# MIT-SPARK/Khronos

Hardware: AMD Instinct MI355X
Metric: active-window frames/sec (+ Mvoxel-updates/sec) at 1280x720 RGB-D+labels, 2 cm voxels (higher is better)
Workload: dtype f32

## Files before the change

### khronos_amd/csrc/khr_kernels_objects.h

```cpp
#pragma once
#include "khr_device.h"

namespace khr {

constexpr int kGvWindow = 32766;
constexpr uint32_t kGvMaxGroup = 32766;
constexpr uint32_t kNodeNone = 0xffffffffu, kNodeOwner = 0x80000000u;

__host__ __device__ inline uint64_t gvKey(uint32_t group, int rx, int ry, int rz) {
  return (static_cast<uint64_t>(group) << 48) | (static_cast<uint64_t>(static_cast<uint32_t>(rx + 32768) & 0xffffu) << 32) |
         (static_cast<uint64_t>(static_cast<uint32_t>(ry + 32768) & 0xffffu) << 16) |
         static_cast<uint64_t>(static_cast<uint32_t>(rz + 32768) & 0xffffu);
}
__host__ __device__ inline uint64_t gvOriginKey(uint32_t group) { return static_cast<uint64_t>(group) << 48; }
__host__ __device__ inline bool gvIsOrigin(uint64_t k) { return (k & 0xffffffffffffull) == 0ull; }
__host__ __device__ inline void gvUnpack(uint64_t k, uint32_t* group, int* rx, int* ry, int* rz) {
  *group = static_cast<uint32_t>(k >> 48);
  *rx = static_cast<int>((k >> 32) & 0xffffu) - 32768;
  *ry = static_cast<int>((k >> 16) & 0xffffu) - 32768;
  *rz = static_cast<int>(k & 0xffffu) - 32768;
}

struct GvTable {
  uint64_t* keys;
// ... 9 lines not shown
    h = (h + 1) & t.mask;
  }
  return -1;
}
__device__ inline uint32_t gvInsert(const GvTable& t, uint64_t key, bool* claimed) {
  uint32_t h = hashKey(key) & t.mask;
  while (true) {
    const unsigned long long prev = atomicCAS(reinterpret_cast<unsigned long long*>(&t.keys[h]),
                                              static_cast<unsigned long long>(kEmptyKey), static_cast<unsigned long long>(key));
    if (prev == kEmptyKey) { *claimed = true; return h; }
    if (prev == key) { *claimed = false; return h; }
    h = (h + 1) & t.mask;
  }
}

__device__ inline uint32_t gvInsertWave(const GvTable& t, bool has, uint64_t key, bool* claimed) {
  const uint32_t lane = laneId();
  const uint32_t klo = static_cast<uint32_t>(key), khi = static_cast<uint32_t>(key >> 32);
  const uint32_t plo = __shfl_up(klo, 1), phi = __shfl_up(khi, 1);
  const unsigned long long hm = __ballot(has);
  const bool prev_has = lane > 0u && ((hm >> (lane - 1u)) & 1ull);
  const bool start = has && !(prev_has && plo == klo && phi == khi);
  const unsigned long long sm = __ballot(start);
  uint32_t h = 0;
  bool cl = false;
  if (start) h = gvInsert(t, key, &cl);
  *claimed = cl;
  const unsigned long long below = sm & (lane == 63u ? ~0ull : ((2ull << lane) - 1ull));
  const int src = below ? 63 - __clzll(static_cast<long long>(below)) : 0;
  const uint32_t hs = __shfl(h, src);
  return has ? hs : 0u;
}

__global__ __launch_bounds__(256) void k_gv_clear(uint64_t* __restrict__ keys, uint32_t n, uint32_t* __restrict__ counters) {
  const uint32_t i = blockIdx.x * blockDim.x + threadIdx.x;
  if (2 * i + 1 < n) reinterpret_cast<ulonglong2*>(keys)[i] = make_ulonglong2(kEmptyKey, kEmptyKey);
  else if (2 * i < n) keys[2 * i] = kEmptyKey;
  if (i < 4) counters[i] = 0u;
}

__device__ inline void pixelVertex(const DevFrame& f, int i, float* pw) {
  pw[0] = pw[1] = pw[2] = 0.f;
  if (f.range[i] > 0.f) {
    const float d = f.depth[i];
    const int u = i % f.W, v = i / f.W;
    xform(f.Rw, f.tw, ((static_cast<float>(u) - f.cx) / f.fx) * d, ((static_cast<float>(v) - f.cy) / f.fy) * d, d, pw);
  }
}

__device__ inline bool gvVoxelKey(const float* pw, float inv, int3 o, uint32_t group, bool vertex_is_origin, uint64_t* key) {
  const int rx = static_cast<int>(floorf(pw[0] * inv)) - o.x, ry = static_cast<int>(floorf(pw[1] * inv)) - o.y,
            rz = static_cast<int>(floorf(pw[2] * inv)) - o.z;
// ... 21 lines not shown
  return -1;
}

struct ObjAcc {
  uint32_t n_pixels;
  uint32_t first_cm;
  int32_t bmin[3], bmax[3];
  float sum[3];
  uint32_t group;
};

__global__ __launch_bounds__(256) void k_obj_insert3d(DevFrame f, const int32_t* __restrict__ obj_labels, int n_labels,
                                                     float max_range, float inv, int3 origin, GvTable t,
                                                     uint32_t* __restrict__ parent, uint32_t* __restrict__ pix_node,
                                                     uint32_t* __restrict__ flags ,
                                                     uint32_t* __restrict__ owners, uint32_t* __restrict__ n_owners) {
  const int i = blockIdx.x * blockDim.x + threadIdx.x;
  const bool in = i < f.W * f.H;
  bool has = false;
  uint64_t key = 0;
  if (in) {
    const int g = labelRank(obj_labels, n_labels, f.label[i]);
    const float r = f.range[i];
    if (g >= 0 && !(max_range > 0.f && r > max_range)) {
      float pw[3];
      pixelVertex(f, i, pw);
      has = gvVoxelKey(pw, inv, origin, static_cast<uint32_t>(g), !(r > 0.f), &key);
      if (!has) atomicOr(&flags[0], 1u);
    }
  }
  bool claimed;
  const uint32_t h = gvInsertWave(t, has, key, &claimed);
  const uint32_t at = waveAggInc(n_owners, claimed);
  if (claimed) {
    parent[h] = h;
    owners[at] = h;
  }
  if (in) pix_node[i] = has ? (h | (claimed ? kNodeOwner : 0u)) : kNodeNone;
}

__constant__ int8_t c_obj_fwd13[13][3] = {{1, 0, 0},  {0, 1, 0},   {0, 0, 1},  {1, 1, 0},  {-1, 1, 0}, {1, 0, 1}, {-1, 0, 1},
                                          {0, 1, 1},  {0, -1, 1},  {1, 1, 1},  {-1, 1, 1}, {1, -1, 1}, {-1, -1, 1}};

__global__ __launch_bounds__(256) void k_obj_union3d(const uint32_t* __restrict__ owners, const uint32_t* __restrict__ n_owners, GvTable t,
                                                    uint32_t* __restrict__ parent, int n_dirs) {
  const uint32_t total = *n_owners * static_cast<uint32_t>(n_dirs);
  for (uint32_t i = blockIdx.x * blockDim.x + threadIdx.x; i < total; i += gridDim.x * blockDim.x) {
    const uint32_t h = owners[i / n_dirs];
    const int k = static_cast<int>(i % n_dirs);
    const uint64_t key = t.keys[h];
    if (gvIsOrigin(key)) continue;
    uint32_t g;
    int x, y, z;
    gvUnpack(key, &g, &x, &y, &z);
    const int nx = x + c_obj_fwd13[k][0], ny = y + c_obj_fwd13[k][1], nz = z + c_obj_fwd13[k][2];
    if (nx < -kGvWindow || nx > kGvWindow || ny < -kGvWindow || ny > kGvWindow || nz < -kGvWindow || nz > kGvWindow) continue;
    const int hn = gvFind(t, gvKey(g, nx, ny, nz));
    if (hn >= 0) ufUnion(parent, h, static_cast<uint32_t>(hn));
  }
}

__global__ __launch_bounds__(256) void k_obj_roots3d(const uint32_t* __restrict__ owners, const uint32_t* __restrict__ n_owners,
                                                    uint32_t* __restrict__ parent, uint32_t* __restrict__ root_idx,
                                                    uint32_t* __restrict__ n_roots, uint32_t cap, ObjAcc* __restrict__ acc,
                                                    const uint64_t* __restrict__ keys) {
  const uint32_t i = blockIdx.x * blockDim.x + threadIdx.x;
  const bool on = i < *n_owners;
  uint32_t h = 0;
  bool is_root = false;
  if (on) {
    h = owners[i];
    const uint32_t r = ufFind(parent, h);
    is_root = r == h;
    if (!is_root) __atomic_store_n(parent + h, r, __ATOMIC_RELAXED);
  }
  const uint32_t idx = waveAggInc(n_roots, is_root);
  if (is_root) {
    root_idx[h] = idx;
    if (idx < cap) {
      ObjAcc a;
      a.n_pixels = 0;
      a.first_cm = 0xffffffffu;
      for (int d = 0; d < 3; ++d) { a.bmin[d] = INT32_MAX; a.bmax[d] = INT32_MIN; a.sum[d] = 0.f; }
      a.group = static_cast<uint32_t>(keys[h] >> 48);
      acc[idx] = a;
    }
  }
}

__global__ __launch_bounds__(256) void k_gv_release(const uint32_t* __restrict__ slots, const uint32_t* __restrict__ n_slots,
                                                   uint64_t* __restrict__ keys) {
  const uint32_t n = *n_slots;
  for (uint32_t i = blockIdx.x * blockDim.x + threadIdx.x; i < n; i += gridDim.x * blockDim.x) keys[slots[i]] = kEmptyKey;
}

__global__ __launch_bounds__(256) void k_gv_release_publish(const uint32_t* __restrict__ slots, const uint32_t* __restrict__ n_slots,
                                                           uint64_t* __restrict__ keys, uint32_t* __restrict__ done_count,
                                                           const uint32_t* __restrict__ src, volatile uint32_t* __restrict__ dst_host,
                                                           uint32_t rec_words, uint32_t max_recs, volatile uint32_t* __restrict__ ticket_host,
                                                           uint32_t ticket, uint32_t* __restrict__ counters_to_zero) {
  __shared__ uint32_t s_last;
// ... 2 lines not shown
  __syncthreads();
  if (threadIdx.x == 0) {
    __threadfence();
    s_last = atomicAdd(done_count, 1u) == gridDim.x - 1u ? 1u : 0u;
  }
  __syncthreads();
  if (!s_last) return;
  const uint32_t n_words = 4u + min(src[0], max_recs) * rec_words;
  for (uint32_t i = threadIdx.x; i < n_words; i += blockDim.x) dst_host[i] = src[i];
  __threadfence_system();
  __syncthreads();
  if (threadIdx.x < 4) counters_to_zero[threadIdx.x] = 0u;
  if (threadIdx.x == 0) {
    *done_count = 0u;
    *ticket_host = ticket;
    __threadfence_system();
  }
}

__global__ __launch_bounds__(256) void k_obj_init2d(DevFrame f, const int32_t* __restrict__ obj_labels, int n_labels,
                                                   uint32_t* __restrict__ parent, uint32_t* __restrict__ pix_node) {
  const int i = blockIdx.x * blockDim.x + threadIdx.x;
  if (i >= f.W * f.H) return;
  const bool cand = labelRank(obj_labels, n_labels, f.label[i]) >= 0;
  parent[i] = static_cast<uint32_t>(i);
  pix_node[i] = cand ? (static_cast<uint32_t>(i) | kNodeOwner) : kNodeNone;
}

__global__ __launch_bounds__(256) void k_obj_union2d(DevFrame f, const uint32_t* __restrict__ pix_node,
                                                    uint32_t* __restrict__ parent, int full) {
// ... 35 lines not shown
  if (is_root) {
    root_idx[h] = idx;
    if (idx < cap) {
      ObjAcc a;
      a.n_pixels = 0;
      a.first_cm = 0xffffffffu;
      for (int d = 0; d < 3; ++d) { a.bmin[d] = INT32_MAX; a.bmax[d] = INT32_MIN; a.sum[d] = 0.f; }
      a.group = keys3d ? static_cast<uint32_t>(keys3d[h] >> 48)
                       : static_cast<uint32_t>(labelRank(obj_labels, n_labels, label2d[h]));
      acc[idx] = a;
    }
  }
}

constexpr int kObjTile = 32, kObjSlots = 16;
__global__ __launch_bounds__(1024) void k_obj_paint(DevFrame f, const uint32_t* __restrict__ pix_node,
                                                   const uint32_t* __restrict__ parent, const uint32_t* __restrict__ root_idx,
                                                   uint32_t cap, int32_t* __restrict__ obj, ObjAcc* __restrict__ acc) {
  __shared__ int s_id[kObjSlots];
  __shared__ ObjAcc s_acc[kObjSlots];
  if (threadIdx.x < kObjSlots) {
    s_id[threadIdx.x] = 0;
    ObjAcc a;
    a.n_pixels = 0;
    a.first_cm = 0xffffffffu;
    for (int d = 0; d < 3; ++d) { a.bmin[d] = INT32_MAX; a.bmax[d] = INT32_MIN; a.sum[d] = 0.f; }
    a.group = 0;
    s_acc[threadIdx.x] = a;
  }
  __syncthreads();
  const int tiles_x = (f.W + kObjTile - 1) / kObjTile;
  const int u = (blockIdx.x % tiles_x) * kObjTile + (threadIdx.x & 31), v = (blockIdx.x / tiles_x) * kObjTile + (threadIdx.x >> 5);
  int id = 0;
  float pw[3] = {0.f, 0.f, 0.f};
  uint32_t cm = 0xffffffffu;
  if (u < f.W && v < f.H) {
    const int i = v * f.W + u;
    const uint32_t node = pix_node[i];
    if (node != kNodeNone) {
      const uint32_t idx = root_idx[ufFind(parent, node & ~kNodeOwner)];
      if (idx < cap) {
        id = static_cast<int>(idx) + 1;
        pixelVertex(f, i, pw);
        cm = static_cast<uint32_t>(u) * static_cast<uint32_t>(f.H) + static_cast<uint32_t>(v);
      }
    }
    obj[i] = id;
  }
  unsigned long long todo = __ballot(id != 0);
  while (todo) {
    const int leader = __ffsll(static_cast<long long>(todo)) - 1;
    const int cid = __shfl(id, leader);
    const bool mine = id == cid;
    const unsigned long long grp = __ballot(mine);
    todo &= ~grp;
    float mn[3], mx[3], sm[3];
    uint32_t first = mine ? cm : 0xffffffffu;
#pragma unroll
    for (int c = 0; c < 3; ++c) {
      mn[c] = mine ? pw[c] : 3.0e38f;
      mx[c] = mine ? pw[c] : -3.0e38f;
      sm[c] = mine ? pw[c] : 0.f;
// ... 37 lines not shown
#pragma unroll
    for (int c = 0; c < 3; ++c) {
      atomicMin(&a->bmin[c], l.bmin[c]);
      atomicMax(&a->bmax[c], l.bmax[c]);
      atomicAdd(&a->sum[c], l.sum[c]);
    }
  }
}

__global__ __launch_bounds__(256) void k_obj_remap(int32_t* __restrict__ obj, int n, const int32_t* __restrict__ final_id) {
  const int i = blockIdx.x * blockDim.x + threadIdx.x;
  if (i >= n) return;
  const int32_t t = obj[i];
  if (t) obj[i] = final_id[t - 1];
}
constexpr int kRemapTab = 256;
struct RemapTab {
  int32_t v[kRemapTab];
};
__global__ __launch_bounds__(256) void k_obj_remap_tab(int32_t* __restrict__ obj, int n, RemapTab tab) {
  __shared__ int32_t s_tab[kRemapTab];
  s_tab[threadIdx.x] = tab.v[threadIdx.x];
  __syncthreads();
  const int i = blockIdx.x * blockDim.x + threadIdx.x;
  if (i >= n) return;
  const int32_t t = obj[i];
  if (t) obj[i] = s_tab[t - 1];
}

__global__ __launch_bounds__(256) void k_cluster_voxels(DevFrame f, const int32_t* __restrict__ id_image, float inv, int3 origin,
                                                       GvTable t, uint64_t* __restrict__ list, uint32_t* __restrict__ n_list,
// ... 46 lines not shown
          pixelVertex(f, i, pw);
          has = gvVoxelKey(pw, inv, origin, static_cast<uint32_t>(id), !(f.range[i] > 0.f), &key);
          if (!has) atomicOr(&flags[0], 1u);
        }
      }
    }
  }
  bool claimed;
  const uint32_t h = gvInsertWave(t, has, key, &claimed);
  const uint32_t at = waveAggInc(n_list, claimed);
  if (claimed && at < cap) {
    list[at] = key;
    slots[at] = h;
  }
}


constexpr int kPixRefs = 32;
struct PixRefs {
  int n;
  int32_t id[kPixRefs];
  int32_t bit[kPixRefs];
};
struct PixCamera {
  double T[12];
  float fx, fy, cx, cy;
  int W, H;
};
__global__ __launch_bounds__(256) void k_pix_reproject(DevFrame src, const int32_t* __restrict__ id_img, PixRefs refs, PixCamera cam,
                                                      uint32_t* __restrict__ mask, uint32_t* __restrict__ n_points) {
  const int i = blockIdx.x * blockDim.x + threadIdx.x;
// ... 169 lines not shown
```

### khronos_amd/csrc/khronos_amd.hip

```cpp
#include <hip/hip_runtime.h>
#include <hip/hip_ext.h>
#include <hipcub/hipcub.hpp>

#include <algorithm>
#include <array>
#include <atomic>
#include <chrono>
#include <memory>
#include <mutex>
#include <cmath>
#include <cstdarg>
#include <cstdio>
#include <climits>
#include <cstring>
#include <cstdlib>
#include <functional>
#include <map>
#include <string>
#include <thread>
#include <tuple>
#include <unordered_map>
#include <vector>

#include "../../include/khronos_amd.h"
// ... 69 lines not shown
  bool dyn_clean = false;
  bool dynw_valid = false;
  uint64_t aux_seq = 0;
  std::vector<khr_cluster> sem_clusters;
  std::vector<khr_cluster> clusters;
};

struct TimingRec {
  int which;
  Event a, b;
};

constexpr int kNumTimers = 13;
constexpr uint32_t kObjHead = 512;
constexpr uint32_t kCvHead = 8192;
constexpr int kGvReleaseGrid = 64;
constexpr uint32_t kCompCap = 1024, kCompHead = 64;

}

struct khr_ctx {
  khr_config cfg{};
  DevParams p{};
  DevMap m{};
  int device = 0;
  Stream stream;
  Stream aux_stream;
  Stream copy_stream;
  Stream snap_stream;
  Stream mc_stream;
// ... 172 lines not shown
  size_t cub_temp_bytes = 0;
  bool obj_configured = false;
  khr_object_detector_config obj_cfg{};
  std::vector<int32_t> obj_labels;
  DevBuf<int32_t> d_obj_labels;
  uint64_t* d_gv_keys = nullptr;
  uint32_t gv_mask = 0;
  uint32_t *d_gv_parent = nullptr, *d_gv_rootidx = nullptr, *d_gv_node = nullptr;
  uint32_t* d_gv_n = nullptr;
  ObjAcc* d_obj_acc = nullptr;
  int32_t* d_obj_final = nullptr;
  uint64_t* d_cv_list = nullptr;
  uint32_t obj_root_cap = 0;
  uint32_t* d_gv_owners = nullptr;
  uint32_t* d_gv_done = nullptr;
  bool gv_clean = false;
  bool gv_counters_clean[4] = {false, false, false, false};
  PinnedBuf<uint8_t> h_obj_head;
  Event ev_obj;
  int obj_pending_slot = -1;
  uint32_t* d_cv_n[3] = {nullptr, nullptr, nullptr};
  uint64_t* d_cv_keys[3] = {nullptr, nullptr, nullptr};
  PinnedBuf<uint8_t> h_cv[3];
  Event ev_cv[3];
  int cv_pending_slot[2] = {-1, -1};
  uint32_t obj_ticket = 0, cv_ticket[3] = {0, 0, 0};
  int3 cv_origin[3]{};
  int cv_set_obj = 1;
  float obj_cv_size = 0.f;
  int obj_cv_slot = -1;
// ... 2507 lines not shown

static int ensureGv(khr_ctx* c) {
  if (c->d_gv_keys) return KHR_OK;
  const size_t npx = c->cfg.max_frame_pixels;
  size_t ts = 1024;
  while (ts < 2 * npx) ts <<= 1;
  c->gv_mask = static_cast<uint32_t>(ts - 1);
  c->obj_root_cap = 1u << 16;
  int rc = KHR_OK;
  KHR_CHAIN(devAlloc(c, &c->d_gv_keys, ts, false));
  KHR_CHAIN(devAlloc(c, &c->d_gv_parent, ts, false));
  KHR_CHAIN(devAlloc(c, &c->d_gv_rootidx, ts, false));
  KHR_CHAIN(devAlloc(c, &c->d_gv_node, npx, false));
  KHR_CHAIN(devAlloc(c, &c->d_gv_owners, npx, false));
  KHR_CHAIN(devAlloc(c, &c->d_gv_done, 4));
  {
    uint8_t* head = nullptr;
    KHR_CHAIN(devAlloc(c, &head, 16 + sizeof(ObjAcc) * c->obj_root_cap));
    c->d_gv_n = reinterpret_cast<uint32_t*>(head);
    c->d_obj_acc = head ? reinterpret_cast<ObjAcc*>(head + 16) : nullptr;
  }
  KHR_CHAIN(devAlloc(c, &c->d_obj_final, c->obj_root_cap, false));
  for (int w = 0; w < 3; ++w) {
    uint8_t* head = nullptr;
    KHR_CHAIN(devAlloc(c, &head, 16 + sizeof(uint64_t) * npx));
    c->d_cv_n[w] = reinterpret_cast<uint32_t*>(head);
    c->d_cv_keys[w] = head ? reinterpret_cast<uint64_t*>(head + 16) : nullptr;
    KHR_CHAIN(c->h_cv[w].alloc(16 + sizeof(uint64_t) * npx));
    KHR_CHAIN(c->ev_cv[w].ensure());
  }
// ... 20 lines not shown
  std::sort(c->obj_labels.begin(), c->obj_labels.end());
  c->obj_labels.erase(std::unique(c->obj_labels.begin(), c->obj_labels.end()), c->obj_labels.end());
  if (c->obj_labels.size() > kGvMaxGroup) return fail(KHR_EINVAL, "more than %u object labels", kGvMaxGroup);
  c->obj_cfg.object_labels = nullptr;
  c->obj_cfg.n_object_labels = static_cast<int32_t>(c->obj_labels.size());
  if (c->d_obj_labels) HIP_TRY(hipStreamSynchronize(c->stream));
  KHR_TRY(c->d_obj_labels.alloc(std::max<size_t>(c->obj_labels.size(), 1)));
  if (!c->obj_labels.empty()) {
    HIP_TRY(hipMemcpyAsync(c->d_obj_labels, c->obj_labels.data(), sizeof(int32_t) * c->obj_labels.size(), hipMemcpyHostToDevice, c->stream));
    HIP_TRY(hipStreamSynchronize(c->stream));
  }
  c->obj_configured = true;
  return KHR_OK;
}

static int objectsLaunch(khr_ctx* c, int slot) {
  FrameSlot& s = c->slots[slot];
  const int n = s.sensor.width * s.sensor.height;
  const khr_object_detector_config& oc = c->obj_cfg;
  s.sem_clusters.clear();
  s.objects_done = false;
  s.has_obj = true;
  s.aux_seq = c->obj_seq = ++c->aux_seq_issued;
  c->obj_pending_slot = -1;
  if (c->obj_cv_slot == slot) c->obj_cv_slot = -1;
  const int n_labels = static_cast<int>(c->obj_labels.size());
  if (!s.has_label || n_labels == 0) {
    HIP_TRY(hipMemsetAsync(s.obj, 0, sizeof(int32_t) * n, c->aux_stream));
    s.objects_done = true;
    return KHR_OK;
  }
  const DevFrame f = makeDevFrame(c, s);
  GvTable t{c->d_gv_keys, c->gv_mask};
  const uint32_t tsize = c->gv_mask + 1;
  if (oc.use_3d) {
    const float inv = 1.f / oc.grid_size;
    if (!c->gv_clean) hipLaunchKernelGGL(k_gv_clear, dim3(gridFor(tsize / 2)), dim3(256), 0, c->aux_stream, c->d_gv_keys, tsize, c->d_gv_n);
    else if (!c->gv_counters_clean[0]) HIP_TRY(hipMemsetAsync(c->d_gv_n, 0, sizeof(uint32_t) * 4, c->aux_stream));
    c->gv_clean = false;
    c->gv_counters_clean[0] = false;
    hipLaunchKernelGGL(k_obj_insert3d, dim3(gridFor(n)), dim3(256), 0, c->aux_stream, f, c->d_obj_labels, n_labels, oc.max_range, inv,
                       windowOrigin(f, inv), t, c->d_gv_parent, c->d_gv_node, c->d_gv_n + 1, c->d_gv_owners, c->d_gv_n + 2);
    hipLaunchKernelGGL(k_obj_union3d, dim3(1024), dim3(256), 0, c->aux_stream, c->d_gv_owners, c->d_gv_n + 2, t, c->d_gv_parent,
                       oc.use_full_connectivity ? 13 : 3);
    hipLaunchKernelGGL(k_obj_roots3d, dim3(gridFor(n)), dim3(256), 0, c->aux_stream, c->d_gv_owners, c->d_gv_n + 2, c->d_gv_parent,
                       c->d_gv_rootidx, c->d_gv_n, c->obj_root_cap, c->d_obj_acc, c->d_gv_keys);
  } else {
    HIP_TRY(hipMemsetAsync(c->d_gv_n, 0, sizeof(uint32_t) * 4, c->aux_stream));
    hipLaunchKernelGGL(k_obj_init2d, dim3(gridFor(n)), dim3(256), 0, c->aux_stream, f, c->d_obj_labels, n_labels, c->d_gv_parent, c->d_gv_node);
    hipLaunchKernelGGL(k_obj_union2d, dim3(gridFor(n)), dim3(256), 0, c->aux_stream, f, c->d_gv_node, c->d_gv_parent,
                       oc.use_full_connectivity ? 1 : 0);
    hipLaunchKernelGGL(k_obj_roots, dim3(gridFor(n)), dim3(256), 0, c->aux_stream, c->d_gv_node, n, c->d_gv_parent, c->d_gv_rootidx, c->d_gv_n,
                       c->obj_root_cap, c->d_obj_acc, nullptr, s.vLabel(), c->d_obj_labels, n_labels);
  }
  const int obj_tiles = ((s.sensor.width + kObjTile - 1) / kObjTile) * ((s.sensor.height + kObjTile - 1) / kObjTile);
  hipLaunchKernelGGL(k_obj_paint, dim3(obj_tiles), dim3(1024), 0, c->aux_stream, f, c->d_gv_node, c->d_gv_parent, c->d_gv_rootidx,
                     c->obj_root_cap, s.obj, c->d_obj_acc);
  HIP_TRY(hipGetLastError());
  if (++c->obj_ticket == 0) ++c->obj_ticket;
  if (oc.use_3d) {
    hipLaunchKernelGGL(k_gv_release_publish, dim3(kGvReleaseGrid), dim3(256), 0, c->aux_stream, c->d_gv_owners, c->d_gv_n + 2, c->d_gv_keys,
                       c->d_gv_done, c->d_gv_n, reinterpret_cast<uint32_t*>(c->h_obj_head.dev()), static_cast<uint32_t>(sizeof(ObjAcc) / 4), kObjHead,
                       c->h_pinned.dev() + 4, c->obj_ticket, c->d_gv_n);
    c->gv_clean = true;
  } else {
    hipLaunchKernelGGL(k_publish, dim3(1), dim3(1024), 0, c->aux_stream, c->d_gv_n, reinterpret_cast<uint32_t*>(c->h_obj_head.dev()),
                       static_cast<uint32_t>(sizeof(ObjAcc) / 4), kObjHead, c->h_pinned.dev() + 4, c->obj_ticket, c->d_gv_n);
  }
  HIP_TRY(hipGetLastError());
  c->gv_counters_clean[0] = oc.use_3d != 0;
  c->obj_pending_slot = slot;
  return KHR_OK;
}

static int cvTicketWord(int set) { return set == 2 ? 12 : 5 + set; }

static int cvReleasePublish(khr_ctx* c, int set) {
  c->gv_clean = true;
  if (++c->cv_ticket[set] == 0) ++c->cv_ticket[set];
  hipLaunchKernelGGL(k_gv_release_publish, dim3(kGvReleaseGrid), dim3(256), 0, c->aux_stream, c->d_gv_owners, c->d_cv_n[set], c->d_gv_keys,
                     c->d_gv_done, c->d_cv_n[set], reinterpret_cast<uint32_t*>(c->h_cv[set].dev()), 2u,
                     static_cast<uint32_t>(std::min<size_t>(kCvHead, c->cfg.max_frame_pixels)), c->h_pinned.dev() + cvTicketWord(set),
                     c->cv_ticket[set], c->d_cv_n[set]);
  HIP_TRY(hipGetLastError());
  c->gv_counters_clean[1 + set] = true;
  return KHR_OK;
}

static int objectsFinish(khr_ctx* c, int slot) {
  FrameSlot& s = c->slots[slot];
  if (s.objects_done) return static_cast<int>(s.sem_clusters.size());
  if (c->obj_pending_slot != slot) return fail(KHR_ESTATE, "object detection was not launched for this slot");
  c->obj_pending_slot = -1;
  const int n = s.sensor.width * s.sensor.height;
  const khr_object_detector_config& oc = c->obj_cfg;
  {
    const int rcw = waitTicket(c, 4, c->obj_ticket, "the object detector's cluster records", c->aux_stream);
    if (rcw) return rcw;
    c->aux_seq_done = std::max(c->aux_seq_done, c->obj_seq);
  }
  const uint32_t* cnt = reinterpret_cast<const uint32_t*>(c->h_obj_head.get());
  if (cnt[1] & 1u) return fail(KHR_EINVAL, "object detector: a measured point lies more than %d grid cells from the sensor", kGvWindow);
  const uint32_t R = cnt[0];
  if (R > c->obj_root_cap) return fail(KHR_ENOMEM, "object detector: %u clusters exceed the capacity %u", R, c->obj_root_cap);
  s.objects_done = true;
  if (R == 0) return 0;
  if (R > kObjHead) {
    HIP_TRY(hipMemcpyAsync(c->h_obj_head, c->d_gv_n, 16 + sizeof(ObjAcc) * R, hipMemcpyDeviceToHost, c->aux_stream));
    HIP_TRY(hipStreamSynchronize(c->aux_stream));
  }
  const ObjAcc* acc = reinterpret_cast<const ObjAcc*>(c->h_obj_head + 16);
  std::vector<uint32_t> order(R);
  for (uint32_t i = 0; i < R; ++i) order[i] = i;
  std::sort(order.begin(), order.end(), [&](uint32_t a, uint32_t b) {
    if (oc.use_3d && acc[a].group != acc[b].group) return acc[a].group < acc[b].group;
    return acc[a].first_cm < acc[b].first_cm;
  });
  std::vector<int32_t> fin(R, 0);
  int next_id = 1;
  for (uint32_t r : order) {
    const ObjAcc& a = acc[r];
// ... 7 lines not shown
      if (size < oc.min_cluster_size) continue;
    }
    fin[r] = id;
    khr_cluster k{};
    k.id = id;
    k.num_pixels_listed = a.n_pixels;
    k.num_pixels_painted = a.n_pixels;
    for (int d = 0; d < 3; ++d) {
      k.bbox_min[d] = orderedToFloat(a.bmin[d]);
      k.bbox_max[d] = orderedToFloat(a.bmax[d]);
      k.centroid[d] = a.sum[d] / static_cast<float>(a.n_pixels);
    }
    k.semantic_id = c->obj_labels[a.group];
    s.sem_clusters.push_back(k);
  }
  if (R <= static_cast<uint32_t>(kRemapTab)) {
    RemapTab tab{};
    std::memcpy(tab.v, fin.data(), sizeof(int32_t) * R);
    if (c->obj_cv_size > 0.f) {
      const int set = 3 - c->cv_set_obj;
      const DevFrame f = makeDevFrame(c, s);
      const float inv = 1.f / c->obj_cv_size;
      s.aux_seq = c->cv_seq[set] = ++c->aux_seq_issued;
      c->cv_origin[set] = windowOrigin(f, inv);
      GvTable t{c->d_gv_keys, c->gv_mask};
      const uint32_t tsize = c->gv_mask + 1;
      if (!c->gv_clean) hipLaunchKernelGGL(k_gv_clear, dim3(gridFor(tsize / 2)), dim3(256), 0, c->aux_stream, c->d_gv_keys, tsize, c->d_cv_n[set]);
      else if (!c->gv_counters_clean[1 + set]) HIP_TRY(hipMemsetAsync(c->d_cv_n[set], 0, sizeof(uint32_t) * 4, c->aux_stream));
      c->gv_clean = false;
      c->gv_counters_clean[1 + set] = false;
      hipLaunchKernelGGL(k_obj_remap_cluster_voxels, dim3(gridFor(n)), dim3(256), 0, c->aux_stream, f, s.obj, tab, inv, c->cv_origin[set], t,
                         c->d_cv_keys[set], c->d_cv_n[set], static_cast<uint32_t>(c->cfg.max_frame_pixels), c->d_cv_n[set] + 1, c->d_gv_owners);
      HIP_TRY(hipGetLastError());
      const int rcp = cvReleasePublish(c, set);
      if (rcp) return rcp;
      c->obj_cv_slot = slot;
    } else {
      hipLaunchKernelGGL(k_obj_remap_tab, dim3(gridFor(n)), dim3(256), 0, c->aux_stream, s.obj, n, tab);
    }
  } else {
    std::memcpy(c->h_obj_head, fin.data(), sizeof(int32_t) * R);
    HIP_TRY(hipMemcpyAsync(c->d_obj_final, c->h_obj_head, sizeof(int32_t) * R, hipMemcpyHostToDevice, c->aux_stream));
// ... 41 lines not shown
int khr_configure_object_voxel_sets(khr_ctx* c, float voxel_size) {
  if (!c) return fail(KHR_EINVAL, "null ctx");
  if (!(voxel_size >= 0.f) || !std::isfinite(voxel_size)) return fail(KHR_EINVAL, "voxel_size must be >= 0 (0 = off)");
  if (voxel_size != c->obj_cv_size) c->obj_cv_slot = -1;
  c->obj_cv_size = voxel_size;
  return KHR_OK;
}

int khr_cluster_voxels_launch(khr_ctx* c, int slot, int which, float voxel_size) {
  if (!c || slot < 0 || slot >= static_cast<int>(c->slots.size()) || !c->slots[slot].valid) return fail(KHR_EINVAL, "bad slot");
  if (!(voxel_size > 0.f) || (which != 0 && which != 1)) return fail(KHR_EINVAL, "bad argument");
  HIP_TRY(hipSetDevice(c->device));
  int rc = ensureGv(c);
  if (rc) return rc;
  FrameSlot& s = c->slots[slot];
  c->cv_pending_slot[which] = slot;
  if (which == 1 && c->obj_cv_slot == slot && c->obj_cv_size == voxel_size && s.has_obj) {
    c->cv_set_obj = 3 - c->cv_set_obj;
    c->obj_cv_slot = -1;
    return KHR_OK;
  }
  const int set = which == 0 ? 0 : c->cv_set_obj;
  uint32_t* hc = reinterpret_cast<uint32_t*>(c->h_cv[set].get());
  if (which == 1 && !s.has_obj) {
    hc[0] = hc[1] = 0;
    c->cv_ticket[set] = c->h_pinned[cvTicketWord(set)];
    return KHR_OK;
  }
  const int n = s.sensor.width * s.sensor.height;
  const DevFrame f = makeDevFrame(c, s);
  const float inv = 1.f / voxel_size;
  if (which == 0) {
    rc = auxAfterMain(c);
    if (rc) return rc;
  }
  s.aux_seq = c->cv_seq[set] = ++c->aux_seq_issued;
  c->cv_origin[set] = windowOrigin(f, inv);
  GvTable t{c->d_gv_keys, c->gv_mask};
  const uint32_t tsize = c->gv_mask + 1;
  if (!c->gv_clean) hipLaunchKernelGGL(k_gv_clear, dim3(gridFor(tsize / 2)), dim3(256), 0, c->aux_stream, c->d_gv_keys, tsize, c->d_cv_n[set]);
  else if (!c->gv_counters_clean[1 + set]) HIP_TRY(hipMemsetAsync(c->d_cv_n[set], 0, sizeof(uint32_t) * 4, c->aux_stream));
  c->gv_clean = false;
  c->gv_counters_clean[1 + set] = false;
  hipLaunchKernelGGL(k_cluster_voxels, dim3(gridFor(n)), dim3(256), 0, c->aux_stream, f, which == 0 ? s.dyn : s.obj, inv, c->cv_origin[set], t,
                     c->d_cv_keys[set], c->d_cv_n[set], static_cast<uint32_t>(c->cfg.max_frame_pixels), c->d_cv_n[set] + 1,
                     c->d_gv_owners);
  HIP_TRY(hipGetLastError());
  return cvReleasePublish(c, set);
}

int64_t khr_cluster_voxels_fetch(khr_ctx* c, int which, int32_t* ids_out, int64_t* voxels_out, int64_t cap) {
  if (!c || (which != 0 && which != 1) || cap < 0 || (cap > 0 && (!ids_out || !voxels_out))) return fail(KHR_EINVAL, "bad argument");
  if (c->cv_pending_slot[which] < 0) return fail(KHR_ESTATE, "khr_cluster_voxels_launch has not been called");
  const int set = which == 0 ? 0 : c->cv_set_obj;
  {
// ... 2637 lines not shown
```

Baseline: 4145.

## Fuse object cluster filtering and voxel-set construction into device-side object pipeline

Object segmentation now computes per-cluster pixel counts and first column-major indices on the device during insertion and root finding. A last-block step in the roots kernel then applies the size filters and assigns final ids on the GPU. The paint kernel builds the per-object voxel set directly into a second hash table, and one combined release/publish kernel replaces the separate cluster-voxel pass. This removes the host round trip and the extra remap and cluster kernels when the object voxel size is configured, at the cost of more atomics, extra buffers and more complex state tracking.

```diff
diff --git a/khronos_amd/csrc/khr_kernels_objects.h b/khronos_amd/csrc/khr_kernels_objects.h
--- a/khronos_amd/csrc/khr_kernels_objects.h
+++ b/khronos_amd/csrc/khr_kernels_objects.h
@@ -47,7 +47,8 @@
   }
 }
 
-__device__ inline uint32_t gvInsertWave(const GvTable& t, bool has, uint64_t key, bool* claimed) {
+__device__ inline uint32_t gvInsertWave(const GvTable& t, bool has, uint64_t key, bool* claimed, bool* run_start = nullptr,
+                                        uint32_t* run_end = nullptr) {
   const uint32_t lane = laneId();
   const uint32_t klo = static_cast<uint32_t>(key), khi = static_cast<uint32_t>(key >> 32);
   const uint32_t plo = __shfl_up(klo, 1), phi = __shfl_up(khi, 1);
@@ -62,13 +63,29 @@
   const unsigned long long below = sm & (lane == 63u ? ~0ull : ((2ull << lane) - 1ull));
   const int src = below ? 63 - __clzll(static_cast<long long>(below)) : 0;
   const uint32_t hs = __shfl(h, src);
+  if (run_end) {
+    const unsigned long long stops = (sm | ~hm) & (lane == 63u ? 0ull : ~((2ull << lane) - 1ull));
+    *run_start = start;
+    *run_end = stops ? static_cast<uint32_t>(__ffsll(static_cast<long long>(stops)) - 1) : 64u;
+  }
   return has ? hs : 0u;
 }
 
-__global__ __launch_bounds__(256) void k_gv_clear(uint64_t* __restrict__ keys, uint32_t n, uint32_t* __restrict__ counters) {
+struct GvPix {
+  uint32_t* count;
+  uint32_t* first_cm;
+};
+
+__global__ __launch_bounds__(256) void k_gv_clear(uint64_t* __restrict__ keys, uint32_t n, uint32_t* __restrict__ counters, GvPix px) {
   const uint32_t i = blockIdx.x * blockDim.x + threadIdx.x;
   if (2 * i + 1 < n) reinterpret_cast<ulonglong2*>(keys)[i] = make_ulonglong2(kEmptyKey, kEmptyKey);
   else if (2 * i < n) keys[2 * i] = kEmptyKey;
+  if (px.count) {
+    for (uint32_t k = 2 * i; k < n && k < 2 * i + 2; ++k) {
+      px.count[k] = 0u;
+      px.first_cm[k] = 0xffffffffu;
+    }
+  }
   if (i < 4) counters[i] = 0u;
 }
 
@@ -120,7 +137,7 @@
                                                      float max_range, float inv, int3 origin, GvTable t,
                                                      uint32_t* __restrict__ parent, uint32_t* __restrict__ pix_node,
                                                      uint32_t* __restrict__ flags ,
-                                                     uint32_t* __restrict__ owners, uint32_t* __restrict__ n_owners) {
+                                                     uint32_t* __restrict__ owners, uint32_t* __restrict__ n_owners, GvPix px) {
   const int i = blockIdx.x * blockDim.x + threadIdx.x;
   const bool in = i < f.W * f.H;
   bool has = false;
@@ -135,8 +152,22 @@
       if (!has) atomicOr(&flags[0], 1u);
     }
   }
-  bool claimed;
-  const uint32_t h = gvInsertWave(t, has, key, &claimed);
+  bool claimed, run_start;
+  uint32_t run_end;
+  const uint32_t h = gvInsertWave(t, has, key, &claimed, &run_start, &run_end);
+  if (px.count) {
+    const uint32_t lane = laneId();
+    uint32_t cm = has ? static_cast<uint32_t>(i % f.W) * static_cast<uint32_t>(f.H) + static_cast<uint32_t>(i / f.W) : 0xffffffffu;
+#pragma unroll
+    for (int o = 1; o < 64; o <<= 1) {
+      const uint32_t other = static_cast<uint32_t>(__shfl_down(static_cast<int>(cm), o));
+      if (lane + static_cast<uint32_t>(o) < run_end) cm = min(cm, other);
+    }
+    if (has && run_start) {
+      atomicAdd(&px.count[h], run_end - lane);
+      atomicMin(&px.first_cm[h], cm);
+    }
+  }
   const uint32_t at = waveAggInc(n_owners, claimed);
   if (claimed) {
     parent[h] = h;
@@ -166,31 +197,88 @@
   }
 }
 
+constexpr int kRemapTab = 256;
 __global__ __launch_bounds__(256) void k_obj_roots3d(const uint32_t* __restrict__ owners, const uint32_t* __restrict__ n_owners,
                                                     uint32_t* __restrict__ parent, uint32_t* __restrict__ root_idx,
                                                     uint32_t* __restrict__ n_roots, uint32_t cap, ObjAcc* __restrict__ acc,
-                                                    const uint64_t* __restrict__ keys) {
-  const uint32_t i = blockIdx.x * blockDim.x + threadIdx.x;
-  const bool on = i < *n_owners;
-  uint32_t h = 0;
-  bool is_root = false;
-  if (on) {
-    h = owners[i];
-    const uint32_t r = ufFind(parent, h);
-    is_root = r == h;
-    if (!is_root) __atomic_store_n(parent + h, r, __ATOMIC_RELAXED);
-  }
-  const uint32_t idx = waveAggInc(n_roots, is_root);
-  if (is_root) {
-    root_idx[h] = idx;
-    if (idx < cap) {
-      ObjAcc a;
-      a.n_pixels = 0;
-      a.first_cm = 0xffffffffu;
-      for (int d = 0; d < 3; ++d) { a.bmin[d] = INT32_MAX; a.bmax[d] = INT32_MIN; a.sum[d] = 0.f; }
-      a.group = static_cast<uint32_t>(keys[h] >> 48);
-      acc[idx] = a;
-    }
+                                                    const uint64_t* __restrict__ keys, GvPix px, uint32_t* __restrict__ root_slot,
+                                                    int32_t* __restrict__ final_id, uint32_t* __restrict__ done_count,
+                                                    int min_size, int max_size) {
+  const uint32_t n = *n_owners;
+  for (uint32_t base = blockIdx.x * blockDim.x; base < n; base += gridDim.x * blockDim.x) {
+    const uint32_t i = base + threadIdx.x;
+    const bool on = i < n;
+    uint32_t h = 0, r = kNodeNone;
+    bool is_root = false;
+    if (on) {
+      h = owners[i];
+      r = ufFind(parent, h);
+      is_root = r == h;
+      if (!is_root) __atomic_store_n(parent + h, r, __ATOMIC_RELAXED);
+    }
+    if (px.count) {
+      const bool fold = on && !is_root;
+      const uint32_t my_n = fold ? px.count[h] : 0u, my_first = fold ? px.first_cm[h] : 0xffffffffu;
+      unsigned long long todo = __ballot(fold);
+      while (todo) {
+        const int leader = __ffsll(static_cast<long long>(todo)) - 1;
+        const uint32_t lr = static_cast<uint32_t>(__shfl(static_cast<int>(r), leader));
+        const bool mine = fold && r == lr;
+        todo &= ~__ballot(mine);
+        uint32_t sum = mine ? my_n : 0u, first = mine ? my_first : 0xffffffffu;
+#pragma unroll
+        for (int o = 32; o > 0; o >>= 1) {
+          sum += static_cast<uint32_t>(__shfl_xor(static_cast<int>(sum), o));
+          first = min(first, static_cast<uint32_t>(__shfl_xor(static_cast<int>(first), o)));
+        }
+        if (static_cast<int>(laneId()) == leader) {
+          atomicAdd(&px.count[lr], sum);
+          atomicMin(&px.first_cm[lr], first);
+        }
+      }
+    }
+    const uint32_t idx = waveAggInc(n_roots, is_root);
+    if (is_root) {
+      root_idx[h] = idx;
+      if (px.count && idx < static_cast<uint32_t>(kRemapTab)) root_slot[idx] = h;
+      if (idx < cap) {
+        ObjAcc a;
+        a.n_pixels = 0;
+        a.first_cm = 0xffffffffu;
+        for (int d = 0; d < 3; ++d) { a.bmin[d] = INT32_MAX; a.bmax[d] = INT32_MIN; a.sum[d] = 0.f; }
+        a.group = static_cast<uint32_t>(keys[h] >> 48);
+        acc[idx] = a;
+      }
+    }
+  }
+  if (!px.count) return;
+  __shared__ uint32_t s_last;
+  __shared__ uint64_t s_key[kRemapTab];
+  __threadfence();
+  __syncthreads();
+  if (threadIdx.x == 0) {
+    __threadfence();
+    s_last = atomicAdd(done_count, 1u) == gridDim.x - 1u ? 1u : 0u;
+  }
+  __syncthreads();
+  if (!s_last) return;
+  __threadfence();
+  if (threadIdx.x == 0) *done_count = 0u;
+  const uint32_t R = __atomic_load_n(n_roots, __ATOMIC_RELAXED);
+  if (R > static_cast<uint32_t>(kRemapTab)) return;
+  uint64_t mine = ~0ull;
+  if (threadIdx.x < R) {
+    const uint32_t h = __atomic_load_n(root_slot + threadIdx.x, __ATOMIC_RELAXED);
+    const int size = static_cast<int>(__atomic_load_n(px.count + h, __ATOMIC_RELAXED));
+    const uint32_t first = __atomic_load_n(px.first_cm + h, __ATOMIC_RELAXED);
+    if (!(size < min_size || (max_size > 0 && size > max_size))) mine = ((keys[h] >> 48) << 32) | first;
+  }
+  s_key[threadIdx.x] = mine;
+  __syncthreads();
+  if (threadIdx.x < R) {
+    int before = 0;
+    for (uint32_t j = 0; j < R; ++j) before += s_key[j] < mine ? 1 : 0;
+    final_id[threadIdx.x] = mine == ~0ull ? 0 : before + 1;
   }
 }
 
@@ -223,6 +311,47 @@
   if (threadIdx.x == 0) {
     *done_count = 0u;
     *ticket_host = ticket;
+    __threadfence_system();
+  }
+}
+
+__global__ __launch_bounds__(256) void k_obj_release_publish(const uint32_t* __restrict__ slots, const uint32_t* __restrict__ n_slots,
+                                                            uint64_t* __restrict__ keys, GvPix px, const uint32_t* __restrict__ cv_slots,
+                                                            uint32_t cv_cap, uint64_t* __restrict__ cv_keys, uint32_t* __restrict__ done_count,
+                                                            uint32_t* __restrict__ obj_src, volatile uint32_t* __restrict__ obj_host,
+                                                            uint32_t obj_rec_words, uint32_t obj_max_recs,
+                                                            volatile uint32_t* __restrict__ obj_ticket_host, uint32_t obj_ticket,
+                                                            uint32_t* __restrict__ cv_src, volatile uint32_t* __restrict__ cv_host,
+                                                            uint32_t cv_max_recs, volatile uint32_t* __restrict__ cv_ticket_host,
+                                                            uint32_t cv_ticket) {
+  __shared__ uint32_t s_last;
+  const uint32_t n = *n_slots, n_cv = min(cv_src[0], cv_cap);
+  for (uint32_t i = blockIdx.x * blockDim.x + threadIdx.x; i < n; i += gridDim.x * blockDim.x) {
+    const uint32_t h = slots[i];
+    keys[h] = kEmptyKey;
+    px.count[h] = 0u;
+    px.first_cm[h] = 0xffffffffu;
+  }
+  for (uint32_t i = blockIdx.x * blockDim.x + threadIdx.x; i < n_cv; i += gridDim.x * blockDim.x) cv_keys[cv_slots[i]] = kEmptyKey;
+  __syncthreads();
+  if (threadIdx.x == 0) {
+    __threadfence();
+    s_last = atomicAdd(done_count, 1u) == gridDim.x - 1u ? 1u : 0u;
+  }
+  __syncthreads();
+  if (!s_last) return;
+  const uint32_t obj_words = 4u + min(obj_src[0], obj_max_recs) * obj_rec_words;
+  for (uint32_t i = threadIdx.x; i < obj_words; i += blockDim.x) obj_host[i] = obj_src[i];
+  const uint32_t cv_words = 4u + min(cv_src[0], cv_max_recs) * 2u;
+  for (uint32_t i = threadIdx.x; i < cv_words; i += blockDim.x) cv_host[i] = cv_src[i];
+  __threadfence_system();
+  __syncthreads();
+  if (threadIdx.x < 4) obj_src[threadIdx.x] = 0u;
+  else if (threadIdx.x < 8) cv_src[threadIdx.x - 4] = 0u;
+  if (threadIdx.x == 0) {
+    *done_count = 0u;
+    *obj_ticket_host = obj_ticket;
+    *cv_ticket_host = cv_ticket;
     __threadfence_system();
   }
 }
@@ -288,11 +417,30 @@
 }
 
 constexpr int kObjTile = 32, kObjSlots = 16;
+struct ObjSets {
+  const int32_t* final_id;
+  const uint32_t* n_roots;
+  float inv;
+  int3 origin;
+  GvTable t;
+  uint64_t* list;
+  uint32_t* n_list;
+  uint32_t cap;
+  uint32_t* flags;
+  uint32_t* slots;
+};
+template <bool SETS>
 __global__ __launch_bounds__(1024) void k_obj_paint(DevFrame f, const uint32_t* __restrict__ pix_node,
                                                    const uint32_t* __restrict__ parent, const uint32_t* __restrict__ root_idx,
-                                                   uint32_t cap, int32_t* __restrict__ obj, ObjAcc* __restrict__ acc) {
+                                                   uint32_t cap, int32_t* __restrict__ obj, ObjAcc* __restrict__ acc, ObjSets sets) {
   __shared__ int s_id[kObjSlots];
   __shared__ ObjAcc s_acc[kObjSlots];
+  __shared__ int32_t s_tab[SETS ? kRemapTab : 1];
+  bool provisional = true;
+  if (SETS) {
+    provisional = *sets.n_roots > static_cast<uint32_t>(kRemapTab);
+    if (!provisional && threadIdx.x < kRemapTab) s_tab[threadIdx.x] = sets.final_id[threadIdx.x];
+  }
   if (threadIdx.x < kObjSlots) {
     s_id[threadIdx.x] = 0;
     ObjAcc a;
@@ -308,18 +456,42 @@
   int id = 0;
   float pw[3] = {0.f, 0.f, 0.f};
   uint32_t cm = 0xffffffffu;
+  bool has = false;
+  uint64_t key = 0;
   if (u < f.W && v < f.H) {
     const int i = v * f.W + u;
     const uint32_t node = pix_node[i];
+    int32_t out = 0;
     if (node != kNodeNone) {
       const uint32_t idx = root_idx[ufFind(parent, node & ~kNodeOwner)];
       if (idx < cap) {
         id = static_cast<int>(idx) + 1;
         pixelVertex(f, i, pw);
         cm = static_cast<uint32_t>(u) * static_cast<uint32_t>(f.H) + static_cast<uint32_t>(v);
-      }
-    }
-    obj[i] = id;
+        out = id;
+        if (SETS && !provisional) {
+          out = s_tab[idx];
+          if (out > 0) {
+            if (static_cast<uint32_t>(out) > kGvMaxGroup) {
+              atomicOr(&sets.flags[0], 2u);
+            } else {
+              has = gvVoxelKey(pw, sets.inv, sets.origin, static_cast<uint32_t>(out), !(f.range[i] > 0.f), &key);
+              if (!has) atomicOr(&sets.flags[0], 1u);
+            }
+          }
+        }
+      }
+    }
+    obj[i] = out;
+  }
+  if (SETS) {
+    bool claimed;
+    const uint32_t h = gvInsertWave(sets.t, has, key, &claimed);
+    const uint32_t at = waveAggInc(sets.n_list, claimed);
+    if (claimed && at < sets.cap) {
+      sets.list[at] = key;
+      sets.slots[at] = h;
+    }
   }
   unsigned long long todo = __ballot(id != 0);
   while (todo) {
@@ -387,7 +559,6 @@
   const int32_t t = obj[i];
   if (t) obj[i] = final_id[t - 1];
 }
-constexpr int kRemapTab = 256;
 struct RemapTab {
   int32_t v[kRemapTab];
 };
@@ -464,7 +635,6 @@
     slots[at] = h;
   }
 }
-
 
 constexpr int kPixRefs = 32;
 struct PixRefs {
diff --git a/khronos_amd/csrc/khronos_amd.hip b/khronos_amd/csrc/khronos_amd.hip
--- a/khronos_amd/csrc/khronos_amd.hip
+++ b/khronos_amd/csrc/khronos_amd.hip
@@ -107,6 +107,7 @@
 constexpr int kNumTimers = 13;
 constexpr uint32_t kObjHead = 512;
 constexpr uint32_t kCvHead = 8192;
+constexpr int kGvRootsGrid = 64;
 constexpr int kGvReleaseGrid = 64;
 constexpr uint32_t kCompCap = 1024, kCompHead = 64;
 
@@ -309,6 +310,12 @@
   uint32_t obj_root_cap = 0;
   uint32_t* d_gv_owners = nullptr;
   uint32_t* d_gv_done = nullptr;
+  uint32_t *d_gv_px_count = nullptr, *d_gv_px_first = nullptr;
+  uint32_t* d_obj_root_slot = nullptr;
+  uint64_t* d_gv2_keys = nullptr;
+  uint32_t* d_gv2_slots = nullptr;
+  bool obj_sets_launched = false;
+  float obj_sets_size = 0.f;
   bool gv_clean = false;
   bool gv_counters_clean[4] = {false, false, false, false};
   PinnedBuf<uint8_t> h_obj_head;
@@ -2846,6 +2853,12 @@
   KHR_CHAIN(devAlloc(c, &c->d_gv_node, npx, false));
   KHR_CHAIN(devAlloc(c, &c->d_gv_owners, npx, false));
   KHR_CHAIN(devAlloc(c, &c->d_gv_done, 4));
+  KHR_CHAIN(devAlloc(c, &c->d_gv_px_count, ts, false));
+  KHR_CHAIN(devAlloc(c, &c->d_gv_px_first, ts, false));
+  KHR_CHAIN(devAlloc(c, &c->d_obj_root_slot, static_cast<size_t>(kRemapTab)));
+  KHR_CHAIN(devAlloc(c, &c->d_gv2_keys, ts, false));
+  KHR_CHAIN(devAlloc(c, &c->d_gv2_slots, npx, false));
+  if (rc == KHR_OK && hipMemsetAsync(c->d_gv2_keys, 0xff, sizeof(uint64_t) * ts, c->stream) != hipSuccess) rc = KHR_EDEVICE;
   {
     uint8_t* head = nullptr;
     KHR_CHAIN(devAlloc(c, &head, 16 + sizeof(ObjAcc) * c->obj_root_cap));
@@ -2896,6 +2909,8 @@
   return KHR_OK;
 }
 
+static int cvTicketWord(int set) { return set == 2 ? 12 : 5 + set; }
+
 static int objectsLaunch(khr_ctx* c, int slot) {
   FrameSlot& s = c->slots[slot];
   const int n = s.sensor.width * s.sensor.height;
@@ -2905,6 +2920,7 @@
   s.has_obj = true;
   s.aux_seq = c->obj_seq = ++c->aux_seq_issued;
   c->obj_pending_slot = -1;
+  c->obj_sets_launched = false;
   if (c->obj_cv_slot == slot) c->obj_cv_slot = -1;
   const int n_labels = static_cast<int>(c->obj_labels.size());
   if (!s.has_label || n_labels == 0) {
@@ -2915,18 +2931,32 @@
   const DevFrame f = makeDevFrame(c, s);
   GvTable t{c->d_gv_keys, c->gv_mask};
   const uint32_t tsize = c->gv_mask + 1;
+  const bool with_sets = oc.use_3d && c->obj_cv_size > 0.f && c->obj_cv_slot < 0;
+  const GvPix px = with_sets ? GvPix{c->d_gv_px_count, c->d_gv_px_first} : GvPix{nullptr, nullptr};
+  ObjSets sets{};
+  const int set = 3 - c->cv_set_obj;
+  if (with_sets) {
+    const float inv_cv = 1.f / c->obj_cv_size;
+    c->cv_seq[set] = c->obj_seq;
+    c->cv_origin[set] = windowOrigin(f, inv_cv);
+    if (!c->gv_counters_clean[1 + set]) HIP_TRY(hipMemsetAsync(c->d_cv_n[set], 0, sizeof(uint32_t) * 4, c->aux_stream));
+    c->gv_counters_clean[1 + set] = false;
+    sets = ObjSets{c->d_obj_final, c->d_gv_n, inv_cv, c->cv_origin[set], GvTable{c->d_gv2_keys, c->gv_mask}, c->d_cv_keys[set], c->d_cv_n[set],
+                   static_cast<uint32_t>(c->cfg.max_frame_pixels), c->d_cv_n[set] + 1, c->d_gv2_slots};
+  }
   if (oc.use_3d) {
     const float inv = 1.f / oc.grid_size;
-    if (!c->gv_clean) hipLaunchKernelGGL(k_gv_clear, dim3(gridFor(tsize / 2)), dim3(256), 0, c->aux_stream, c->d_gv_keys, tsize, c->d_gv_n);
+    if (!c->gv_clean) hipLaunchKernelGGL(k_gv_clear, dim3(gridFor(tsize / 2)), dim3(256), 0, c->aux_stream, c->d_gv_keys, tsize, c->d_gv_n, GvPix{c->d_gv_px_count, c->d_gv_px_first});
     else if (!c->gv_counters_clean[0]) HIP_TRY(hipMemsetAsync(c->d_gv_n, 0, sizeof(uint32_t) * 4, c->aux_stream));
     c->gv_clean = false;
     c->gv_counters_clean[0] = false;
     hipLaunchKernelGGL(k_obj_insert3d, dim3(gridFor(n)), dim3(256), 0, c->aux_stream, f, c->d_obj_labels, n_labels, oc.max_range, inv,
-                       windowOrigin(f, inv), t, c->d_gv_parent, c->d_gv_node, c->d_gv_n + 1, c->d_gv_owners, c->d_gv_n + 2);
+                       windowOrigin(f, inv), t, c->d_gv_parent, c->d_gv_node, c->d_gv_n + 1, c->d_gv_owners, c->d_gv_n + 2, px);
     hipLaunchKernelGGL(k_obj_union3d, dim3(1024), dim3(256), 0, c->aux_stream, c->d_gv_owners, c->d_gv_n + 2, t, c->d_gv_parent,
                        oc.use_full_connectivity ? 13 : 3);
-    hipLaunchKernelGGL(k_obj_roots3d, dim3(gridFor(n)), dim3(256), 0, c->aux_stream, c->d_gv_owners, c->d_gv_n + 2, c->d_gv_parent,
-                       c->d_gv_rootidx, c->d_gv_n, c->obj_root_cap, c->d_obj_acc, c->d_gv_keys);
+    hipLaunchKernelGGL(k_obj_roots3d, dim3(kGvRootsGrid), dim3(256), 0, c->aux_stream, c->d_gv_owners, c->d_gv_n + 2, c->d_gv_parent,
+                       c->d_gv_rootidx, c->d_gv_n, c->obj_root_cap, c->d_obj_acc, c->d_gv_keys, px, c->d_obj_root_slot, c->d_obj_final,
+                       c->d_gv_done + 1, oc.min_cluster_size, oc.max_cluster_size);
   } else {
     HIP_TRY(hipMemsetAsync(c->d_gv_n, 0, sizeof(uint32_t) * 4, c->aux_stream));
     hipLaunchKernelGGL(k_obj_init2d, dim3(gridFor(n)), dim3(256), 0, c->aux_stream, f, c->d_obj_labels, n_labels, c->d_gv_parent, c->d_gv_node);
@@ -2936,11 +2966,27 @@
                        c->obj_root_cap, c->d_obj_acc, nullptr, s.vLabel(), c->d_obj_labels, n_labels);
   }
   const int obj_tiles = ((s.sensor.width + kObjTile - 1) / kObjTile) * ((s.sensor.height + kObjTile - 1) / kObjTile);
-  hipLaunchKernelGGL(k_obj_paint, dim3(obj_tiles), dim3(1024), 0, c->aux_stream, f, c->d_gv_node, c->d_gv_parent, c->d_gv_rootidx,
-                     c->obj_root_cap, s.obj, c->d_obj_acc);
+  if (with_sets)
+    hipLaunchKernelGGL(k_obj_paint<true>, dim3(obj_tiles), dim3(1024), 0, c->aux_stream, f, c->d_gv_node, c->d_gv_parent, c->d_gv_rootidx,
+                       c->obj_root_cap, s.obj, c->d_obj_acc, sets);
+  else
+    hipLaunchKernelGGL(k_obj_paint<false>, dim3(obj_tiles), dim3(1024), 0, c->aux_stream, f, c->d_gv_node, c->d_gv_parent, c->d_gv_rootidx,
+                       c->obj_root_cap, s.obj, c->d_obj_acc, sets);
   HIP_TRY(hipGetLastError());
   if (++c->obj_ticket == 0) ++c->obj_ticket;
-  if (oc.use_3d) {
+  if (with_sets) {
+    if (++c->cv_ticket[set] == 0) ++c->cv_ticket[set];
+    hipLaunchKernelGGL(k_obj_release_publish, dim3(kGvReleaseGrid), dim3(256), 0, c->aux_stream, c->d_gv_owners, c->d_gv_n + 2, c->d_gv_keys, px,
+                       c->d_gv2_slots, static_cast<uint32_t>(c->cfg.max_frame_pixels), c->d_gv2_keys, c->d_gv_done, c->d_gv_n,
+                       reinterpret_cast<uint32_t*>(c->h_obj_head.dev()), static_cast<uint32_t>(sizeof(ObjAcc) / 4), kObjHead, c->h_pinned.dev() + 4,
+                       c->obj_ticket, c->d_cv_n[set], reinterpret_cast<uint32_t*>(c->h_cv[set].dev()),
+                       static_cast<uint32_t>(std::min<size_t>(kCvHead, c->cfg.max_frame_pixels)), c->h_pinned.dev() + cvTicketWord(set),
+                       c->cv_ticket[set]);
+    c->gv_clean = true;
+    c->gv_counters_clean[1 + set] = true;
+    c->obj_sets_launched = true;
+    c->obj_sets_size = c->obj_cv_size;
+  } else if (oc.use_3d) {
     hipLaunchKernelGGL(k_gv_release_publish, dim3(kGvReleaseGrid), dim3(256), 0, c->aux_stream, c->d_gv_owners, c->d_gv_n + 2, c->d_gv_keys,
                        c->d_gv_done, c->d_gv_n, reinterpret_cast<uint32_t*>(c->h_obj_head.dev()), static_cast<uint32_t>(sizeof(ObjAcc) / 4), kObjHead,
                        c->h_pinned.dev() + 4, c->obj_ticket, c->d_gv_n);
@@ -2954,8 +3000,6 @@
   c->obj_pending_slot = slot;
   return KHR_OK;
 }
-
-static int cvTicketWord(int set) { return set == 2 ? 12 : 5 + set; }
 
 static int cvReleasePublish(khr_ctx* c, int set) {
   c->gv_clean = true;
@@ -2986,7 +3030,10 @@
   const uint32_t R = cnt[0];
   if (R > c->obj_root_cap) return fail(KHR_ENOMEM, "object detector: %u clusters exceed the capacity %u", R, c->obj_root_cap);
   s.objects_done = true;
-  if (R == 0) return 0;
+  if (R == 0) {
+    if (c->obj_sets_launched && c->obj_sets_size == c->obj_cv_size) c->obj_cv_slot = slot;
+    return 0;
+  }
   if (R > kObjHead) {
     HIP_TRY(hipMemcpyAsync(c->h_obj_head, c->d_gv_n, 16 + sizeof(ObjAcc) * R, hipMemcpyDeviceToHost, c->aux_stream));
     HIP_TRY(hipStreamSynchronize(c->aux_stream));
@@ -3024,6 +3071,10 @@
     k.semantic_id = c->obj_labels[a.group];
     s.sem_clusters.push_back(k);
   }
+  if (c->obj_sets_launched && R <= static_cast<uint32_t>(kRemapTab)) {
+    if (c->obj_sets_size == c->obj_cv_size) c->obj_cv_slot = slot;
+    return static_cast<int>(s.sem_clusters.size());
+  }
   if (R <= static_cast<uint32_t>(kRemapTab)) {
     RemapTab tab{};
     std::memcpy(tab.v, fin.data(), sizeof(int32_t) * R);
@@ -3035,7 +3086,7 @@
       c->cv_origin[set] = windowOrigin(f, inv);
       GvTable t{c->d_gv_keys, c->gv_mask};
       const uint32_t tsize = c->gv_mask + 1;
-      if (!c->gv_clean) hipLaunchKernelGGL(k_gv_clear, dim3(gridFor(tsize / 2)), dim3(256), 0, c->aux_stream, c->d_gv_keys, tsize, c->d_cv_n[set]);
+      if (!c->gv_clean) hipLaunchKernelGGL(k_gv_clear, dim3(gridFor(tsize / 2)), dim3(256), 0, c->aux_stream, c->d_gv_keys, tsize, c->d_cv_n[set], GvPix{c->d_gv_px_count, c->d_gv_px_first});
       else if (!c->gv_counters_clean[1 + set]) HIP_TRY(hipMemsetAsync(c->d_cv_n[set], 0, sizeof(uint32_t) * 4, c->aux_stream));
       c->gv_clean = false;
       c->gv_counters_clean[1 + set] = false;
@@ -3107,6 +3158,10 @@
   int rc = ensureGv(c);
   if (rc) return rc;
   FrameSlot& s = c->slots[slot];
+  if (which == 1 && c->obj_pending_slot == slot) {
+    const int ns = objectsFinish(c, slot);
+    if (ns < 0) return ns;
+  }
   c->cv_pending_slot[which] = slot;
   if (which == 1 && c->obj_cv_slot == slot && c->obj_cv_size == voxel_size && s.has_obj) {
     c->cv_set_obj = 3 - c->cv_set_obj;
@@ -3131,7 +3186,7 @@
   c->cv_origin[set] = windowOrigin(f, inv);
   GvTable t{c->d_gv_keys, c->gv_mask};
   const uint32_t tsize = c->gv_mask + 1;
-  if (!c->gv_clean) hipLaunchKernelGGL(k_gv_clear, dim3(gridFor(tsize / 2)), dim3(256), 0, c->aux_stream, c->d_gv_keys, tsize, c->d_cv_n[set]);
+  if (!c->gv_clean) hipLaunchKernelGGL(k_gv_clear, dim3(gridFor(tsize / 2)), dim3(256), 0, c->aux_stream, c->d_gv_keys, tsize, c->d_cv_n[set], GvPix{c->d_gv_px_count, c->d_gv_px_first});
   else if (!c->gv_counters_clean[1 + set]) HIP_TRY(hipMemsetAsync(c->d_cv_n[set], 0, sizeof(uint32_t) * 4, c->aux_stream));
   c->gv_clean = false;
   c->gv_counters_clean[1 + set] = false;
```

After: 4013. 0.968x the previous value.
